# TheMTank/GridUniverse

Hardware: AMD Instinct MI355X
Metric: env-steps/sec at N_envs on 32×32 grid, 1/2/4/8 MI355X; bit-exact vs CPU (higher is better)
Workload: dtype int32; 1 GPU; c3: 65536 envs per GPU on the 32x32 generator maze (random.seed(123); np.random.seed(123)), uniform device-RNG actions, auto-reset, 1000 env-steps per launch, int32 (obs,reward,done) rows; envs_per_gpu=65536, env_steps_per_launch=1000, global_envs=65536, parallelism=env-index shards, no data-path collective

## Files before the change

### griduniverse_amd/csrc/gu_map.hpp

```cpp
#pragma once
#include "gu_internal.hpp"
#include "gu_rng.hpp"

#define GU_BLOCK 256

struct CellMap {
    const uint8_t *f;
    const int8_t *r;
};

__device__ __forceinline__ uint32_t gu_block_grid(const GridSel &gs)
{
    if (gs.n_grids <= 1) return 0u;
    const int64_t first = (int64_t)blockIdx.x * blockDim.x + (gs.per_wave ? (int64_t)(threadIdx.x & ~63u) : 0);
    const int64_t grid = first / gs.group;
    return (uint32_t)(grid < gs.n_grids ? grid : gs.n_grids - 1);
}

template <bool LDS>
__device__ __forceinline__ CellMap gu_stage_map(const uint8_t *__restrict__ g, int32_t cell_bytes, uint8_t *smem, const GridSel &gs,
                                                int planes = 2)
{
    if (LDS) {
        g += (int64_t)gu_block_grid(gs) * gs.grid_stride;
        if (gs.per_wave) {
            smem += (threadIdx.x >> 6) * (uint32_t)(planes * cell_bytes);
            for (int32_t i = (threadIdx.x & 63) * 16; i < planes * cell_bytes; i += 64 * 16)
                *reinterpret_cast<uint4 *>(smem + i) = *reinterpret_cast<const uint4 *>(g + i);
        } else {
            for (int32_t i = threadIdx.x * 16; i < planes * cell_bytes; i += blockDim.x * 16)
                *reinterpret_cast<uint4 *>(smem + i) = *reinterpret_cast<const uint4 *>(g + i);
        }
        __syncthreads();
        return CellMap{smem, reinterpret_cast<const int8_t *>(smem + cell_bytes)};
    }
    return CellMap{g, reinterpret_cast<const int8_t *>(g + cell_bytes)};
}

struct LaneGrid {
    const int32_t *starts;
    uint32_t n_starts;
};

template <bool LDS>
__device__ __forceinline__ LaneGrid gu_lane_grid(const GridSel &gs, const int32_t *starts, uint32_t n_starts0, uint32_t e, CellMap &m)
{
    if (gs.n_grids <= 1) return LaneGrid{starts, n_starts0};
    if (LDS) {
        const uint32_t gb = gu_block_grid(gs);
        return LaneGrid{starts + (int64_t)gb * gs.max_starts, (uint32_t)gs.n_starts[gb]};
    }
    const uint32_t g = e / (uint32_t)gs.group;
    m.f += (int64_t)g * gs.grid_stride;
    m.r += (int64_t)g * gs.grid_stride;
    return LaneGrid{starts + (int64_t)g * gs.max_starts, (uint32_t)gs.n_starts[g]};
}

template <bool LUT>
__device__ __forceinline__ int32_t gu_delta(uint32_t a, uint64_t lut, int32_t W)
{
    if (LUT) return __builtin_amdgcn_sbfe((int32_t)(uint32_t)(lut >> (a << 4)), 0, 16);
    const int32_t sign = (int32_t)(a & 2u) - 1;
    return (a & 1u) ? -sign : sign * W;
}

__device__ __forceinline__ int32_t gu_reward_packed(uint32_t flags)
{
    return __builtin_amdgcn_sbfe((int32_t)0xF6F60AFFu, (flags >> 2) & 24u, 8);
}

__device__ __forceinline__ int32_t gu_move(int32_t s, uint32_t flags, uint32_t a, int32_t delta)
{
    return __mul24((int32_t)__builtin_amdgcn_ubfe(flags, a, 1), delta) + s;
}
```

### griduniverse_amd/csrc/gu_rollout.hpp

```cpp
#pragma once
#include "gu_map.hpp"

#include <cstdlib>
#include <functional>
#include <type_traits>

__device__ __forceinline__ uint32_t gu_sample_action(uint32_t word, const uint4 q)
{
    return (uint32_t)(word >= q.x) + (uint32_t)(word >= q.y) + (uint32_t)(word >= q.z) - q.w;
}


#define GU_DPP_REDUCE(x, OP)                                                                                     \
    do {                                                                                                         \
        uint32_t o_;                                                                                             \
        o_ = (uint32_t)__builtin_amdgcn_update_dpp(0, (int)(x), 0x111, 0xF, 0xF, false), (x) = OP((x), o_);      \
        o_ = (uint32_t)__builtin_amdgcn_update_dpp(0, (int)(x), 0x112, 0xF, 0xF, false), (x) = OP((x), o_);      \
        o_ = (uint32_t)__builtin_amdgcn_update_dpp(0, (int)(x), 0x114, 0xF, 0xF, false), (x) = OP((x), o_);      \
        o_ = (uint32_t)__builtin_amdgcn_update_dpp(0, (int)(x), 0x118, 0xF, 0xF, false), (x) = OP((x), o_);      \
        o_ = (uint32_t)__builtin_amdgcn_update_dpp(0, (int)(x), 0x142, 0xA, 0xF, false), (x) = OP((x), o_);      \
        o_ = (uint32_t)__builtin_amdgcn_update_dpp(0, (int)(x), 0x143, 0xC, 0xF, false), (x) = OP((x), o_);      \
    } while (0)
#define GU_OP_ADD(a_, b_) ((a_) + (b_))
#define GU_OP_MAX(a_, b_) ((a_) > (b_) ? (a_) : (b_))

struct GuPacer {
    uint64_t due, t0;
    uint32_t ticks;
    uint32_t report_at;
    uint32_t n_steps;
    uint32_t p_q;
    uint64_t *slot;
    uint64_t w[16];
    uint32_t c_seq, c_phase, c_left, c_ema_p, c_ema_u, v_period_q, v_seq, v_unpaced, v_report_steps, v_groups;
    uint32_t c_dec_q, c_block_left, c_block_sum, c_block_n, c_last_mean, c_up, c_quiet;
    uint64_t v_t_start;
    bool first_wave;
    __device__ __forceinline__ void fetch(const GuPaceArgs &pa, bool on)
    {
        ticks = on ? pa.period : 0u;
        p_q = pa.period << 6;
        first_wave = false;
        if (on && pa.ring) {
            const GuPaceEntry *entry = pa.ring + (pa.seq & (GU_PACE_RING - 1u));
            const GuPaceEntry *prev = pa.ring + ((pa.seq - 1u) & (GU_PACE_RING - 1u));
            c_seq = entry->seq;
            const bool mine = c_seq == pa.seq;
            const uint32_t have = mine ? entry->period_q : 0u;
            const uint32_t unpaced = mine ? entry->unpaced : 0u;
            c_phase = entry->phase, c_left = entry->left, c_ema_p = entry->ema_paced, c_ema_u = entry->ema_unpaced;
            v_period_q = prev->period_q, v_seq = prev->seq, v_unpaced = prev->unpaced, v_t_start = prev->t_start;
            v_report_steps = prev->report_steps, v_groups = prev->groups;
            if (have && !pa.fixed) p_q = have;
            p_q = p_q < (pa.lo << 6) ? (pa.lo << 6) : p_q;
            p_q = p_q > (pa.hi << 6) ? (pa.hi << 6) : p_q;
            if (pa.fixed) p_q = pa.period << 6;
            ticks = (unpaced && !pa.fixed) ? 0u : (p_q + 32u) >> 6;
            c_quiet = (mine && !pa.fixed) ? entry->quiet : 0u;
            first_wave = blockIdx.x == 0 && __builtin_amdgcn_readfirstlane(threadIdx.x) < 64u;
            if (first_wave && !c_quiet) {
                c_dec_q = entry->dec_q, c_block_left = entry->block_left, c_block_sum = entry->block_sum, c_block_n = entry->block_n;
                c_last_mean = entry->last_mean, c_up = entry->up;
                const uint64_t *set = pa.slots + (size_t)((pa.seq - 1u) & 1u) * pa.slot_stride;
#pragma unroll
                for (uint32_t j = 0; j < 16u; ++j) {
                    const uint32_t i = j * 64u + threadIdx.x;
                    w[j] = i < pa.n_waves ? __builtin_nontemporal_load(set + i) : 0ull;
                }
            }
        }
    }
    __device__ __forceinline__ void start(const GuPaceArgs &pa, bool on)
    {
        slot = nullptr;
        n_steps = 0;
        report_at = 0;
        t0 = 0;
        if (on && pa.ring) {
            const uint64_t now = __builtin_amdgcn_s_memrealtime();
            due = t0 = now;
            if (c_quiet) {
                if (first_wave) decide_quiet(pa, now);
                return;
            }
            const uint32_t wave = __builtin_amdgcn_readfirstlane((blockIdx.x * blockDim.x + threadIdx.x) >> 6);
            slot = pa.slots + (size_t)(pa.seq & 1u) * pa.slot_stride + wave;
            report_at = pa.report_at;
            if (first_wave) decide(pa, now);
            return;
        }
        due = ticks ? __builtin_amdgcn_s_memrealtime() : 0ull;
    }
    __device__ __forceinline__ void decide_early(const GuPaceArgs &pa)
    {
        if (first_wave && !c_quiet) decide(pa, __builtin_amdgcn_s_memrealtime());
    }
    __device__ __forceinline__ void decide_quiet(const GuPaceArgs &pa, uint64_t now)
    {
        first_wave = false;
        if (threadIdx.x == 0) {
            GuPaceEntry *cur = pa.ring + (pa.seq & (GU_PACE_RING - 1u));
            GuPaceEntry *next = pa.ring + ((pa.seq + 1u) & (GU_PACE_RING - 1u));
            uint32_t ema_u = c_ema_u;
            const uint64_t gap = now - v_t_start;
            const uint32_t took = gap > 0x7FFFFFFFull ? 0x7FFFFFFFu : (uint32_t)gap;
            if (v_seq + 1u == pa.seq && v_unpaced && v_t_start && v_groups == pa.groups && (!ema_u || took < 2u * ema_u)) ema_u = ema_u ? (ema_u * 7u + took) >> 3 : took;
            cur->t_start = now, cur->groups = pa.groups, cur->report_steps = 0;
            const uint32_t left = c_left > 0u ? c_left - 1u : 0u;
            next->period_q = p_q, next->seq = pa.seq + 1u, next->t_start = 0, next->unpaced = 1u;
            next->phase = GU_PACE_OFF, next->left = left, next->ema_paced = c_ema_p, next->ema_unpaced = ema_u;
            next->verdict = 0, next->waves = 0, next->elapsed = 0, next->ended_late = 0, next->max_behind = 0, next->report_steps = 0, next->groups = 0;
            next->dec_q = pa.dec_q, next->block_left = GU_PACE_BLOCK, next->block_sum = 0, next->block_n = 0, next->last_mean = 0, next->up = 0;
            next->quiet = left > 1u ? 1u : 0u;
        }
    }
    __device__ __forceinline__ void decide(const GuPaceArgs &pa, uint64_t now)
    {
        first_wave = false;
        uint64_t *set = pa.slots + (size_t)((pa.seq - 1u) & 1u) * pa.slot_stride;
        GuPaceEntry *cur = pa.ring + (pa.seq & (GU_PACE_RING - 1u));
        GuPaceEntry *prev = pa.ring + ((pa.seq - 1u) & (GU_PACE_RING - 1u));
        const bool fresh = c_seq != pa.seq;
        const bool prev_ok = v_seq + 1u == pa.seq;
        const uint32_t prev_ticks = (prev_ok && !v_unpaced) ? (pa.fixed ? pa.period : (v_period_q + 32u) >> 6) : 0u;
        const uint32_t scheduled = (prev_ticks * ((v_report_steps + 15u) & ~15u)) >> 4;
        const bool same_length = v_groups == pa.groups;
        uint32_t counts = 0, most = 0, longest = 0;
        for (uint32_t base = 0; base < pa.n_waves; base += 64u * 16u) {
            if (base) {
#pragma unroll
                for (uint32_t j = 0; j < 16u; ++j) {
                    const uint32_t i = base + j * 64u + threadIdx.x;
                    w[j] = i < pa.n_waves ? __builtin_nontemporal_load(set + i) : 0ull;
                }
            }
#pragma unroll
            for (uint32_t j = 0; j < 16u; ++j) {
                const uint32_t i = base + j * 64u + threadIdx.x;
                if (i < pa.n_waves) set[i] = 0;
                const uint32_t reported = (uint32_t)(w[j] >> 63), elapsed = (uint32_t)w[j] & 0x7FFFFFFFu;
                const uint32_t behind = (prev_ticks && elapsed > scheduled) ? elapsed - scheduled : 0u;
                counts += (reported << 16) + ((reported && behind > 2u * prev_ticks) ? 1u : 0u);
                most = behind > most ? behind : most;
                longest = elapsed > longest ? elapsed : longest;
            }
        }
        GU_DPP_REDUCE(counts, GU_OP_ADD);
        GU_DPP_REDUCE(most, GU_OP_MAX);
        GU_DPP_REDUCE(longest, GU_OP_MAX);
        if (threadIdx.x == 63) {
            const uint32_t waves = counts >> 16, far = counts & 0xFFFFu;
            GuPaceEntry *next = pa.ring + ((pa.seq + 1u) & (GU_PACE_RING - 1u));
            uint32_t n_q = p_q, phase = GU_PACE_NORMAL, left = pa.probe_every ? (pa.probe_every < 128u ? pa.probe_every : 128u) : 0u, ema_p = 0, ema_u = 0;
            uint32_t dec_q = pa.dec_q, block_left = GU_PACE_BLOCK, block_sum = 0, block_n = 0, last_mean = 0, up = 0;
            if (!fresh) {
                phase = c_phase, left = c_left, ema_p = c_ema_p, ema_u = c_ema_u;
                dec_q = c_dec_q, block_left = c_block_left, block_sum = c_block_sum, block_n = c_block_n, last_mean = c_last_mean, up = c_up;
            } else {
                cur->unpaced = 0, cur->phase = phase, cur->left = left, cur->ema_paced = 0, cur->ema_unpaced = 0;
                cur->dec_q = dec_q, cur->block_left = block_left, cur->block_sum = 0, cur->block_n = 0, cur->last_mean = 0, cur->up = up;
            }
            cur->period_q = p_q, cur->seq = pa.seq, cur->t_start = now, cur->report_steps = pa.report_at, cur->groups = pa.groups;
            cur->verdict = 0, cur->waves = 0, cur->elapsed = 0, cur->ended_late = 0, cur->max_behind = 0;
            if (waves && prev_ok) {
                prev->verdict = (uint64_t)most * 256u > (uint64_t)prev_ticks * v_groups * pa.bar_num ? 2u : 1u;
                prev->waves = waves, prev->elapsed = longest, prev->ended_late = far, prev->max_behind = far ? most : 0u;
                const uint64_t gap = now - v_t_start;
                const uint32_t mean = v_unpaced ? ema_u : ema_p;
                const uint32_t took = gap > 0x7FFFFFFFull ? 0x7FFFFFFFu : (uint32_t)gap;
                const bool plausible = same_length && v_t_start && (!mean || took < 2u * mean);
                if (v_unpaced) {
                    if (plausible) ema_u = ema_u ? (ema_u + took) >> 1 : took;
                } else {
                    if (plausible) ema_p = ema_p ? (ema_p * 7u + took) >> 3 : took;
                    const uint32_t step_up = (uint32_t)(((uint64_t)pa.gain_q * far) / waves);
                    const uint32_t early = 512u / (8u + (pa.seq > 100000u ? 100000u : pa.seq));
                    const uint32_t dec = early > dec_q ? early : dec_q;
                    n_q += step_up;
                    n_q = n_q > dec ? n_q - dec : n_q;
                    if (phase == GU_PACE_NORMAL && !pa.fixed && pa.adapt) {
                        if (block_left <= GU_PACE_BLOCK - GU_PACE_BLOCK_SKIP && plausible) block_sum += took, ++block_n;
                        if (block_left) --block_left;
                        if (!block_left) {
                            const uint32_t mean = block_n ? block_sum / block_n : 0u;
                            if (mean && last_mean && mean > last_mean) up ^= 1u;
                            if (mean) last_mean = mean;
                            dec_q = up ? (dec_q * 4u + 2u) / 3u : (dec_q * 3u) / 4u;
                            dec_q = dec_q < 4u ? 4u : dec_q;
                            dec_q = dec_q > pa.gain_q / 8u ? pa.gain_q / 8u : dec_q;
                            block_left = GU_PACE_BLOCK, block_sum = 0, block_n = 0;
                        }
                    }
                }
            }
            n_q = n_q < (pa.lo << 6) ? (pa.lo << 6) : n_q;
            n_q = n_q > (pa.hi << 6) ? (pa.hi << 6) : n_q;
            if (pa.probe_every && !pa.fixed && left && --left == 0u) {
                const bool off_wins = ema_u && ema_p && (uint64_t)ema_u * 100u < (uint64_t)ema_p * 98u;
                if (phase != GU_PACE_NORMAL || off_wins) block_left = GU_PACE_BLOCK, block_sum = 0, block_n = 0, last_mean = 0;
                if (phase == GU_PACE_NORMAL) phase = GU_PACE_PROBE_OFF, left = 4u, ema_u = 0u;
                else if (phase == GU_PACE_OFF) phase = GU_PACE_PROBE_ON, left = 8u, ema_p = 0u;
                else if (off_wins) phase = GU_PACE_OFF, left = 2u * pa.probe_every;
                else phase = GU_PACE_NORMAL, left = pa.probe_every;
            }
            next->period_q = n_q, next->seq = pa.seq + 1u, next->t_start = 0;
            next->unpaced = (phase == GU_PACE_PROBE_OFF || phase == GU_PACE_OFF) ? 1u : 0u;
            next->phase = phase, next->left = left, next->ema_paced = ema_p, next->ema_unpaced = ema_u;
            next->dec_q = dec_q, next->block_left = block_left, next->block_sum = block_sum, next->block_n = block_n, next->last_mean = last_mean, next->up = up;
            next->quiet = (phase == GU_PACE_OFF && left > 1u) ? 1u : 0u;
            next->verdict = 0, next->waves = 0, next->elapsed = 0, next->ended_late = 0, next->max_behind = 0, next->report_steps = 0, next->groups = 0;
        }
    }
    __device__ __forceinline__ void report(uint64_t now)
    {
        if ((threadIdx.x & 63u) == 0u) {
            const uint64_t elapsed = now - t0;
            *slot = (1ull << 63) | (elapsed > 0x7FFFFFFFull ? 0x7FFFFFFFull : elapsed);
        }
        report_at = 0;
    }
    __device__ __forceinline__ bool idle() const { return ticks == 0u && slot == nullptr; }
    __device__ __forceinline__ void after(uint32_t steps)
    {
// ... 27 lines not shown
    uint32_t *episode;
    const uint32_t *tcount;
    const int32_t *starts;
    const uint32_t *actions;
    int32_t *tr_obs, *tr_reward, *tr_done;
    int32_t *ret, *episodes_fin;
    uint64_t *done_bits;
    uint32_t n_starts, seed_prefix, env_id0, steps_taken;
    uint32_t seed_prefix0, steps_hi;
    const uint32_t *nib;
    int32_t nib_dwords;
    uint64_t lut_p;
    int32_t straddle;
    int64_t N, T;
    GridSel gs;
    const uint32_t *rows;
    const uint32_t *rows2;
    int32_t row_shift;
    int32_t stream_lds_off;
    int32_t stream_lds_words;
    int32_t entry_table;
    int32_t half_waves;
    int32_t xcd_remap;
    GuPaceArgs pace;
};

__device__ __forceinline__ uint32_t gu_env_block(int32_t xcd_remap)
{
    const uint32_t b = blockIdx.x;
    return xcd_remap ? (b & 7u) * (gridDim.x >> 3) + (b >> 3) : b;
}

template <bool TAIL16 = false, class S16, class S1>
__device__ __forceinline__ void gu_stream_run(const char *pa, int64_t row, uint32_t e4, int64_t T, int64_t i0, S16 &&step16, S1 &&step1)
{
    const uint32_t row32 = (uint32_t)row;
    auto word_at = [&](int64_t k, uint32_t c) {
        return (uint32_t)__builtin_amdgcn_raw_buffer_load_b32(__builtin_amdgcn_make_buffer_rsrc((void *)(pa + k * row), 0, 0xFFFFFFFFu, 0x00020000), e4,
                                                              c * row32, 0);
    };
    int64_t i = i0, k = i0 >> 4;
    if (i & 15) {
        const uint32_t word = word_at(k, 0);
        for (; i < T && (i & 15); ++i) step1((word >> (2u * (uint32_t)(i & 15))) & 3u);
        ++k;
    }
    uint32_t w[4];
#pragma unroll
    for (uint32_t c = 0; c < 4; ++c) w[c] = word_at(k, c);
    for (const int64_t full = T >> 4; k + 4 <= full; k += 4, i += 64) {
#pragma unroll
        for (uint32_t c = 0; c < 4; ++c) {
            const uint32_t word = w[c];
            asm volatile("" ::"v"(word));
            w[c] = word_at(k + 4, c);
            step16(word);
        }
    }
    uint32_t q = 0;
    if (TAIL16) {
        for (; i + 16 <= T; i += 16, q += 16) {
            const uint32_t sel = q >> 4;
            step16(sel == 0 ? w[0] : sel == 1 ? w[1] : w[2]);
        }
    }
    for (; i < T; ++i, ++q) {
        const uint32_t sel = q >> 4, word = sel == 0 ? w[0] : sel == 1 ? w[1] : sel == 2 ? w[2] : w[3];
        step1((word >> (2u * (q & 15u))) & 3u);
    }
}

#ifndef GU_STORE_AUX
#define GU_STORE_AUX 18
#endif
#ifndef GU_STORE_AUX_PACKED
#define GU_STORE_AUX_PACKED 16
#endif
#define GU_MAX_BLOCK 1024
typedef uint32_t gu_v3u __attribute__((ext_vector_type(3)));
template <int POLICY, int AUTO, int TRAJ, bool STATS, int MAP>
__global__ void __launch_bounds__(GU_MAX_BLOCK) gu_rollout_kernel(const RolloutArgs a)
{
    constexpr bool LDS = MAP == 1 || MAP == 3;
    extern __shared__ __attribute__((aligned(16))) uint8_t smem[];
    GuPacer pacer;
    pacer.fetch(a.pace, TRAJ == 1 || TRAJ == 3);
    const int64_t e64 = (int64_t)gu_env_block(a.xcd_remap) * blockDim.x + threadIdx.x;
    const bool live = e64 < a.N;
    const uint32_t e = (uint32_t)e64;
    int32_t s = 0, r = 0;
    uint32_t d = 0, ep = 0, tcount0 = 0;
    if (live) {
        s = a.pos[e];
        r = a.reward[e];
        d = (uint32_t)a.done[e];
        ep = a.episode[e];
        tcount0 = a.tcount[e];
    }
    CellMap m = gu_stage_map<LDS>(a.cell, a.cell_bytes, smem, a.gs, MAP == 3 ? 1 : 2);
    const uint32_t nib_region = MAP == 5 ? (threadIdx.x >> 6) * (uint32_t)a.nib_dwords * 256u : 0u;
    if (MAP == 5) {
        const size_t wave = ((size_t)blockIdx.x * blockDim.x + threadIdx.x) >> 6;
        const uint4 *src = reinterpret_cast<const uint4 *>(a.nib + wave * (size_t)a.nib_dwords * 64u);
        uint4 *dst = reinterpret_cast<uint4 *>(smem + nib_region);
        if (wave * 64u < (size_t)a.N)
            for (int32_t i = threadIdx.x & 63; i < a.nib_dwords * 16; i += 64) dst[i] = src[i];
        __syncthreads();
    }
    const uint8_t *greedy = a.greedy;
    if (MAP == 1 && POLICY == GU_POLICY_GREEDY) {
        uint8_t *dst = smem + 2 * a.cell_bytes;
        for (int32_t i = threadIdx.x * 16; i < a.cell_bytes; i += blockDim.x * 16)
            *reinterpret_cast<uint4 *>(dst + i) = *reinterpret_cast<const uint4 *>(a.greedy + i);
        __syncthreads();
        greedy = dst;
    }
    const bool thr_in_lds = MAP == 1 && POLICY == GU_POLICY_SAMPLE && a.pi_lds;
    uint4 *thr_lds = reinterpret_cast<uint4 *>(smem + 2 * a.cell_bytes);
    if (thr_in_lds) {
        for (int32_t i = threadIdx.x; i < a.S; i += blockDim.x) thr_lds[i] = a.pi_thr[i];
        __syncthreads();
    }
    if (!live) return;
    LaneGrid lg = gu_lane_grid<LDS>(a.gs, a.starts, a.n_starts, e, m);

    const uint32_t t_lane = tcount0 + a.steps_taken;
    const uint32_t prefix = gu_rng_prefix(a.seed_prefix, a.env_id0 + e);
    const uint32_t prefix0 = AUTO == 2 ? gu_rng_prefix(a.seed_prefix0, a.env_id0 + e) : prefix;
    const uint32_t epoch0 = (uint32_t)((uint64_t)((int64_t)(((uint64_t)a.steps_hi << 32) | a.steps_taken) + (int64_t)(int32_t)tcount0) >> 32);
    auto prefix_at = [&](uint32_t t) {
        return gu_rng_prefix(gu_rng_seed_prefix_epoch(a.seed_prefix0, epoch0 + (t < t_lane ? 1u : 0u)), a.env_id0 + e);
    };
    constexpr uint32_t TERM5 = 0x20u, TERM5_BIT = 5u;
    auto flags5 = [](uint32_t b) { return (((b >> 5) & 3u) << 3) | (((b >> GU_CELL_TERM_BIT) & 1u) << TERM5_BIT) | ((b >> 7) << 6); };
    uint32_t flags = MAP == 5 ? flags5(m.f[s]) : m.f[s];
    int32_t ret = 0, fin = 0;
    const int32_t W = a.W;
    const uint64_t lut = a.lut;
    const int32_t start0 = lg.starts[0];
    const uint32_t start0_flags = MAP == 5 ? flags5(m.f[start0]) : m.f[start0];
    auto padded = [&](int32_t c) { return (int32_t)(((uint32_t)(c + c / W + W + 2) << 5) + nib_region); };
    int32_t sq = MAP == 5 ? padded(s) : 0;
    const int32_t start0_q = MAP == 5 ? padded(start0) : 0;
    typedef __attribute__((address_space(3))) const uint32_t *lds_word_ptr;
    const uint32_t lane4 = (threadIdx.x & 63u) << 2;
    auto word_at = [&](int32_t cq) { return *(lds_word_ptr)(uintptr_t)(((uint32_t)cq & 0xFFFFFF00u) | lane4); };
    auto four_of = [](uint32_t word, int32_t cq) { return __builtin_amdgcn_ubfe(word, (uint32_t)cq >> 3, 4); };
    auto four_at = [&](int32_t cq) { return four_of(word_at(cq), cq); };
    auto cell5 = [&](int32_t cq) { return four_at(cq) << 3; };
    auto move5 = [&](uint32_t act, int32_t delta, auto &&in_the_shadow) {
        int32_t cand = s + delta;
        asm volatile("" : "+v"(cand));
        const int32_t candq = sq + gu_delta<true>(act, a.lut_p, 0);
        const uint32_t word = word_at(candq);
        in_the_shadow();
        const uint32_t four = four_of(word, candq);
        const bool go = ((flags & TERM5) | four) < 8u;
        s = go ? cand : s;
        sq = go ? candq : sq;
        flags = go ? four << 3 : flags;
    };
    char *po = (char *)a.tr_obs, *pr = (char *)a.tr_reward, *pd = (char *)a.tr_done;
    const char *pa = (const char *)a.actions;
    const uint32_t e4 = e * 4u;
    const int64_t row = a.N * 4;
    const uint32_t row32 = (uint32_t)row;
    const int64_t trow = TRAJ == 3 ? a.N * 12 : row;
    const uint32_t trow32 = (uint32_t)trow;
    const uint32_t te = TRAJ == 3 ? e * 12u : e4;
    __amdgpu_buffer_rsrc_t ro = __builtin_amdgcn_make_buffer_rsrc(po, 0, 0xFFFFFFFFu, 0x00020000);
    __amdgpu_buffer_rsrc_t rr = __builtin_amdgcn_make_buffer_rsrc(pr, 0, 0xFFFFFFFFu, 0x00020000);
    __amdgpu_buffer_rsrc_t rd = __builtin_amdgcn_make_buffer_rsrc(pd, 0, 0xFFFFFFFFu, 0x00020000);
    auto emit = [&](int32_t s_, int32_t r_, uint32_t d_, uint32_t soff) {
        if (TRAJ == 1) {
            __builtin_amdgcn_raw_buffer_store_b32(s_, ro, e4, soff, GU_STORE_AUX);
            __builtin_amdgcn_raw_buffer_store_b32(r_, rr, e4, soff, GU_STORE_AUX);
            __builtin_amdgcn_raw_buffer_store_b32((int32_t)d_, rd, e4, soff, GU_STORE_AUX);
        } else if (TRAJ == 2) {
            __builtin_amdgcn_raw_buffer_store_b32((int32_t)((uint32_t)s_ | (((uint32_t)r_ & 0xFFu) << 16) | (d_ << 24)), ro, e4, soff, GU_STORE_AUX_PACKED);
        } else if (TRAJ == 3) {
            const gu_v3u triple = {(uint32_t)s_, (uint32_t)r_, d_};
            __builtin_amdgcn_raw_buffer_store_b96(triple, ro, te, soff, GU_STORE_AUX);
            GU_WIDE_STORE_PAD();
        }
    };
    bool held = false;
    int32_t held_s = 0, held_r = 0;
    uint32_t held_d = 0, held_soff = 0;
    auto release = [&]() {
        if (MAP == 5 && TRAJ && held) emit(held_s, held_r, held_d, held_soff);
        held = false;
    };
    auto rebase = [&](int64_t rows) {
        release();
        po += rows * trow;
        ro = __builtin_amdgcn_make_buffer_rsrc(po, 0, 0xFFFFFFFFu, 0x00020000);
        if (TRAJ == 1) {
            pr += rows * trow;
            pd += rows * trow;
            rr = __builtin_amdgcn_make_buffer_rsrc(pr, 0, 0xFFFFFFFFu, 0x00020000);
            rd = __builtin_amdgcn_make_buffer_rsrc(pd, 0, 0xFFFFFFFFu, 0x00020000);
        }
    };

    if (AUTO == 1 && MAP != 5) flags = (flags & ~GU_CELL_TERM) | (d << GU_CELL_TERM_BIT);

    auto step = [&](uint32_t act, uint32_t soff) {
        const int32_t delta = gu_delta<MAP != 0>(act, lut, W);
        if (AUTO == 1) {
            const bool was_done = MAP == 5 ? d != 0u : (flags & GU_CELL_TERM) != 0u;
            ep += was_done;
            s = was_done ? start0 : s;
            flags = was_done ? start0_flags : flags;
            if (MAP == 5) sq = was_done ? start0_q : sq;
        } else if (AUTO == 2) {
            if (d) {
                s = lg.starts[gu_rng_start_index(prefix0, ep, lg.n_starts)];
                ++ep;
                if (MAP == 5) sq = padded(s);
                flags = MAP == 5 ? cell5(sq) : m.f[s];
            }
        }
        if (MAP == 5) {
            move5(act, delta, [&]() {
                if (TRAJ && held) {
                    __builtin_amdgcn_sched_barrier(0);
                    emit(held_s, held_r, held_d, held_soff);
                    __builtin_amdgcn_sched_barrier(0);
                }
            });
        } else {
            s = gu_move(s, flags, act, delta);
            flags = m.f[s];
        }
        r = MAP == 5 ? __builtin_amdgcn_sbfe((int32_t)0xF6F60AFFu, flags, 8) : (MAP >= 2) ? gu_reward_packed(flags) : (int32_t)m.r[s];
        d = __builtin_amdgcn_ubfe(flags, MAP == 5 ? TERM5_BIT : GU_CELL_TERM_BIT, 1);
        if (STATS) {
            ret += r;
            fin += (int32_t)d;
        }
        if (MAP == 5 && TRAJ) held = true, held_s = s, held_r = r, held_d = d, held_soff = soff;
        else emit(s, r, d, soff);
    };
    auto step1 = [&](uint32_t act) {
        step(act, 0);
        if (TRAJ) rebase(1);
    };

    pacer.start(a.pace, TRAJ == 1 || TRAJ == 3);
    if (POLICY == GU_POLICY_UNIFORM && a.straddle) {
        uint32_t t = t_lane;
#pragma nounroll
        for (int64_t i = 0; i < a.T; ++i, ++t) step1((gu_rng_word(prefix_at(t), GU_RNG_STREAM_ACTION, t >> 4) >> (2u * (t & 15u))) & 3u);
    } else if (POLICY == GU_POLICY_UNIFORM) {
        const uint32_t t_first = __builtin_amdgcn_readfirstlane(t_lane);
        if (__all(t_lane == t_first)) {
            uint32_t t = t_first;
            int64_t i = 0;
            if (t & 15u) {
                const uint32_t word = gu_rng_word(prefix, GU_RNG_STREAM_ACTION, t >> 4);
                for (; i < a.T && (t & 7u); ++i, ++t) step1((word >> (2u * (t & 15u))) & 3u);
                if ((t & 15u) == 8u && i + 8 <= a.T) {
#pragma unroll
                    for (uint32_t j = 0; j < 8; ++j) step(__builtin_amdgcn_ubfe(word, 16 + 2 * j, 2), j * trow32);
                    if (TRAJ) rebase(8);
                    i += 8, t += 8;
                }
                for (; i < a.T && (t & 15u); ++i, ++t) step1((word >> (2u * (t & 15u))) & 3u);
                pacer.after((uint32_t)i);
            }
            for (; i + 16 <= a.T; i += 16, t += 16) {
                uint32_t word = gu_rng_word(prefix, GU_RNG_STREAM_ACTION, t >> 4);
                if (MAP == 5) asm volatile("" : "+v"(word));
#pragma unroll
                for (uint32_t j = 0; j < 16; ++j) step(__builtin_amdgcn_ubfe(word, 2 * j, 2), j * trow32);
                if (TRAJ) rebase(16);
                if (i + 16 < a.T) pacer.after(16);
            }
            if (i < a.T) {
                const uint32_t word = gu_rng_word(prefix, GU_RNG_STREAM_ACTION, t >> 4);
                uint32_t j = 0;
                if (i + 8 <= a.T) {
#pragma unroll
                    for (uint32_t k = 0; k < 8; ++k) step(__builtin_amdgcn_ubfe(word, 2 * k, 2), k * trow32);
                    if (TRAJ) rebase(8);
                    i += 8, j = 8;
                }
                for (; i < a.T; ++i, ++j) step1((word >> (2u * j)) & 3u);
            }
        } else {
            uint32_t t = t_lane;
            uint32_t word = gu_rng_word(prefix, GU_RNG_STREAM_ACTION, t >> 4);
            for (int64_t i = 0; i < a.T; ++i) {
                step1((word >> (2u * (t & 15u))) & 3u);
                ++t;
                if ((t & 15u) == 0u) word = gu_rng_word(prefix, GU_RNG_STREAM_ACTION, t >> 4);
            }
        }
    } else if (POLICY == GU_POLICY_STREAM) {
        const char *pw = pa;
        auto load_word = [&](uint32_t soff) {
            return (uint32_t)__builtin_amdgcn_raw_buffer_load_b32(__builtin_amdgcn_make_buffer_rsrc((void *)pw, 0, 0xFFFFFFFFu, 0x00020000), e4, soff, 0);
        };
        const int64_t KW = (MAP == 1) ? a.stream_lds_words : 0;
        if (KW) {
            uint32_t *sw = reinterpret_cast<uint32_t *>(smem + a.stream_lds_off) + threadIdx.x;
            const uint32_t bd = blockDim.x;
            int64_t words_left = (a.T + 15) >> 4, i = 0;
            while (i < a.T) {
                const int64_t cnt = words_left < KW ? words_left : KW;
                int64_t k = 0;
                for (; k + 8 <= cnt; k += 8) {
                    uint32_t w[8];
#pragma unroll
                    for (int j = 0; j < 8; ++j) w[j] = load_word(j * row32);
#pragma unroll
                    for (int j = 0; j < 8; ++j) sw[(k + j) * bd] = w[j];
                    pw += 8 * row;
                }
                for (; k < cnt; ++k, pw += row) sw[k * bd] = load_word(0);
                words_left -= cnt;
                const int64_t steps = (a.T - i) < cnt * 16 ? (a.T - i) : cnt * 16;
                uint32_t word = sw[0];
                for (k = 0; k * 16 + 16 <= steps; ++k) {
                    const uint32_t next = k + 1 < cnt ? sw[(k + 1) * bd] : 0u;
#pragma unroll
                    for (uint32_t j = 0; j < 16; ++j) step(__builtin_amdgcn_ubfe(word, 2 * j, 2), j * trow32);
                    if (TRAJ) rebase(16);
                    pacer.after(16);
                    word = next;
                }
                for (int64_t q = k * 16, j = 0; q < steps; ++q, ++j) step1((word >> (2u * (uint32_t)j)) & 3u);
// ... 227 lines not shown
```

### griduniverse_amd/csrc/gu_rollout_rows.hip

```cpp
#include "gu_rollout.hpp"

#define GU_ROW_ADDR_MASK 0xFFFFFu
#define GU_ROW_DONE_BIT 23

struct BuildRowsArgs {
    const uint8_t *cell;
    int32_t cell_bytes, S, W, start0, auto_reset, row_shift;
    uint32_t *rows;
};

__global__ void __launch_bounds__(256) gu_build_rows_kernel(const BuildRowsArgs a)
{
    const int32_t s = blockIdx.x * blockDim.x + threadIdx.x;
    if (s >= a.S) return;
    const int32_t base = (a.auto_reset && (a.cell[s] & GU_CELL_TERM)) ? a.start0 : s;
    const uint32_t fb = a.cell[base];
    uint32_t out[4];
#pragma unroll
    for (uint32_t act = 0; act < 4; ++act) {
        const int32_t n = base + (((fb >> act) & 1u) ? gu_delta<false>(act, 0, a.W) : 0);
        const uint32_t d = (a.cell[n] >> GU_CELL_TERM_BIT) & 1u;
        const uint32_t r = (uint8_t)a.cell[a.cell_bytes + n];
        out[act] = ((uint32_t)n << a.row_shift) | (d << GU_ROW_DONE_BIT) | (r << 24);
    }
// ... 15 lines not shown
    const uint32_t d = (cell[n] >> GU_CELL_TERM_BIT) & 1u;
    const uint32_t r = (uint8_t)cell[cell_bytes + n];
    return ((uint32_t)n << row_shift) | (d << GU_ROW_DONE_BIT) | (r << 24);
}

__global__ void __launch_bounds__(256) gu_build_policy_rows_kernel(const BuildPolicyRowsArgs a)
{
    const int32_t s = blockIdx.x * blockDim.x + threadIdx.x;
    if (s >= a.S) return;
    const int32_t base = (a.auto_reset && (a.cell[s] & GU_CELL_TERM)) ? a.start0 : s;
    if (!a.thr) {
        a.rows[s] = gu_row_record(a.cell, a.cell_bytes, base, a.greedy[base], a.W, a.row_shift);
        return;
    }
    uint4 *out = reinterpret_cast<uint4 *>(a.rows + 8 * (int64_t)s);
    const uint4 q = a.thr[base];
    uint32_t t0 = q.x, t1 = q.y, t2 = q.z;
    if (t0 > t1) { const uint32_t x = t0; t0 = t1; t1 = x; }
    if (t1 > t2) { const uint32_t x = t1; t1 = t2; t2 = x; }
    if (t0 > t1) { const uint32_t x = t0; t0 = t1; t1 = x; }
    out[0] = make_uint4(t0, t1, t2, q.w);
    uint32_t rec[4];
#pragma unroll
    for (uint32_t c = 0; c < 4; ++c) {
        const uint32_t act = c >= q.w ? (c - q.w > 3u ? 3u : c - q.w) : 0u;
        rec[c] = gu_row_record(a.cell, a.cell_bytes, base, act, a.W, a.row_shift);
    }
    out[1] = make_uint4(rec[0], rec[1], rec[2], rec[3]);
}

__device__ __forceinline__ uint32_t gu_row_record(const uint8_t *cell, int32_t cell_bytes, int32_t base, uint32_t act, int32_t W, int32_t row_shift);

struct BuildPairRowsArgs {
    const uint8_t *cell;
    int32_t cell_bytes, S, W, start0, auto_reset;
    uint32_t *rows2;
};

#define GU_PAIR_SHIFT 7

__global__ void __launch_bounds__(256) gu_build_pair_rows_kernel(const BuildPairRowsArgs a)
{
    const int32_t idx = blockIdx.x * blockDim.x + threadIdx.x;
    if (idx >= a.S * 16) return;
    const int32_t s = idx >> 4;
    const uint32_t a1 = (uint32_t)idx & 3u, a2 = ((uint32_t)idx >> 2) & 3u;
    const int32_t b1 = (a.auto_reset && (a.cell[s] & GU_CELL_TERM)) ? a.start0 : s;
    const uint32_t r1 = gu_row_record(a.cell, a.cell_bytes, b1, a1, a.W, GU_PAIR_SHIFT);
    const int32_t n1 = (int32_t)((r1 & GU_ROW_ADDR_MASK) >> GU_PAIR_SHIFT);
    const int32_t b2 = (a.auto_reset && (a.cell[n1] & GU_CELL_TERM)) ? a.start0 : n1;
    const uint32_t r2 = gu_row_record(a.cell, a.cell_bytes, b2, a2, a.W, GU_PAIR_SHIFT);
    reinterpret_cast<uint2 *>(a.rows2)[idx] = make_uint2(r1, r2);
}

typedef __attribute__((address_space(3))) const uint32_t *lds_u32_ptr;
typedef uint32_t gu_v2u __attribute__((ext_vector_type(2)));
typedef __attribute__((address_space(3))) const gu_v2u *lds_v2u_ptr;
typedef uint32_t gu_v4u __attribute__((ext_vector_type(4)));
typedef __attribute__((address_space(3))) const gu_v4u *lds_v4u_ptr;

template <int POLICY>
struct RowBytes {
    static constexpr int log2 = POLICY == GU_POLICY_GREEDY ? 2 : POLICY == GU_POLICY_SAMPLE ? 5 : 4;
};

#define GU_CHAIN_FENCE() __builtin_amdgcn_sched_barrier(0)
#define GU_ROWS_MAX_BLOCK 512
template <int POLICY, int TRAJ, bool STATS, bool PAIR = false>
__global__ void __launch_bounds__(GU_ROWS_MAX_BLOCK) gu_rollout_rows_kernel(const RolloutArgs a, const int32_t auto_reset)
{
    static_assert(!PAIR || POLICY == GU_POLICY_UNIFORM || POLICY == GU_POLICY_STREAM, "pair tables: policies whose actions do not depend on the state");
    extern __shared__ __attribute__((aligned(16))) uint8_t smem[];
    GuPacer pacer;
    pacer.fetch(a.pace, TRAJ != 0);
    const int32_t shift = PAIR ? GU_PAIR_SHIFT : a.row_shift;
    const int32_t copies_log2 = shift - RowBytes<POLICY>::log2;
    constexpr uint32_t lds_base = 0u;
    const uint32_t half = (uint32_t)a.half_waves;
    const uint32_t slot_in_block = half ? ((threadIdx.x >> 6) << 5) | (threadIdx.x & 31u) : threadIdx.x;
    const int64_t e64 = (int64_t)gu_env_block(a.xcd_remap) * (blockDim.x >> half) + slot_in_block;
    const bool live = e64 < a.N && !(half && (threadIdx.x & 32u));
    const uint32_t e = live ? (uint32_t)e64 : 0u;
    const uint32_t prefix = gu_rng_prefix(a.seed_prefix, a.env_id0 + e);
    const int32_t start0 = auto_reset ? a.starts[0] : 0;
    const char *pa = (const char *)a.actions;
    const uint32_t e4 = e * 4u;
    int32_t s = 0;
    uint32_t d = 0, ep = 0, t_lane = 0, f0 = 0, first_x = 0, f1 = 0, r1 = 0, first_word = 0;
    uint4 first_thr = make_uint4(0u, 0u, 0u, 0u);
    auto first_0 = [&]() {
        uint32_t ee = e;
        asm volatile("" : "+v"(ee));
        s = a.pos[ee];
        d = (uint32_t)a.done[ee];
        ep = a.episode[ee];
        t_lane = a.tcount[ee];
    };
    const bool entry_table = a.entry_table != 0;
    auto first_a = [&]() {
        asm volatile("" : "+v"(t_lane), "+v"(s), "+v"(d));
        t_lane += a.steps_taken;
        if (POLICY == GU_POLICY_SAMPLE) first_word = gu_rng_sample_word(prefix, t_lane);
        if (auto_reset && d) {
            if (!entry_table) s = start0;
            ++ep;
        }
        if (!entry_table) {
            f0 = a.cell[s];
            if (POLICY == GU_POLICY_GREEDY) first_x = a.greedy[s];
            if (POLICY == GU_POLICY_SAMPLE) first_thr = a.pi_thr[s];
        }
        if (POLICY == GU_POLICY_UNIFORM) first_x = (gu_rng_word(prefix, GU_RNG_STREAM_ACTION, t_lane >> 4) >> (2u * (t_lane & 15u))) & 3u;
        if (POLICY == GU_POLICY_STREAM) first_x = (uint32_t)__builtin_amdgcn_raw_buffer_load_b32(__builtin_amdgcn_make_buffer_rsrc((void *)pa, 0, 0xFFFFFFFFu, 0x00020000), e4, 0, 0) & 3u;
    };
    auto first_b = [&]() {
        if (entry_table) return;
        asm volatile("" : "+v"(f0));
        const uint32_t act = POLICY == GU_POLICY_SAMPLE ? gu_sample_action(first_word, first_thr) : first_x;
        const int8_t *rew = reinterpret_cast<const int8_t *>(a.cell + a.cell_bytes);
        s += ((f0 >> act) & 1u) ? gu_delta<false>(act, 0, a.W) : 0;
        f1 = a.cell[s];
        r1 = (uint32_t)(uint8_t)rew[s];
    };
    {
        uint4 *dst = reinterpret_cast<uint4 *>(smem);
        const uint32_t copies = 1u << copies_log2;
        if (POLICY == GU_POLICY_GREEDY && copies_log2 < 2) {
            const int32_t units = (a.S << shift) >> 4;
            first_0();
            first_a();
#pragma unroll 8
            for (int32_t u = threadIdx.x; u < units; u += blockDim.x) {
                const int32_t d0 = u << 2;
                uint4 v = make_uint4(a.rows[d0 >> copies_log2], a.rows[(d0 + 1) >> copies_log2], a.rows[(d0 + 2) >> copies_log2], a.rows[(d0 + 3) >> copies_log2]);
                v.x += lds_base, v.y += lds_base, v.z += lds_base, v.w += lds_base;
                dst[u] = v;
            }
            first_b();
        } else {
            const int32_t B = (int32_t)blockDim.x, log2_b = 31 - __builtin_clz((uint32_t)B);
            const int32_t n_src = PAIR ? a.S * 9 : POLICY == GU_POLICY_SAMPLE ? 2 * a.S : a.S;
            const uint4 *g4 = reinterpret_cast<const uint4 *>(PAIR ? a.rows2 : a.rows);
            const uint32_t places = PAIR ? 1u : POLICY == GU_POLICY_GREEDY ? copies >> 2 : copies;
            auto put = [&](uint4 v, int32_t g) {
                if (PAIR || (POLICY != GU_POLICY_GREEDY && (POLICY != GU_POLICY_SAMPLE || (g & 1)))) v.x += lds_base, v.y += lds_base, v.z += lds_base, v.w += lds_base;
                if (PAIR) {
                    dst[g] = v;
                    return;
                }
                const uint32_t cell = POLICY == GU_POLICY_SAMPLE ? (uint32_t)g >> 1 : (uint32_t)g;
                auto at = [&](uint32_t k) {
                    const uint32_t place = (k + cell) & (places - 1u);
                    return POLICY == GU_POLICY_SAMPLE ? ((cell * places + place) << 1) | ((uint32_t)g & 1u) : cell * places + place;
                };
                if (places == 8u) {
#pragma unroll
                    for (uint32_t k = 0; k < 8u; ++k) dst[at(k)] = v;
                } else if (places == 4u) {
#pragma unroll
                    for (uint32_t k = 0; k < 4u; ++k) dst[at(k)] = v;
                } else {
                    for (uint32_t k = 0; k < places; ++k) dst[at(k)] = v;
                }
            };
            auto stage = [&](auto nb, int32_t base, auto between) {
                constexpr int NB = decltype(nb)::value;
                uint4 v[NB];
// ... 442 lines not shown
```

### griduniverse_amd/csrc/gu_rollout_uniform.hip

```cpp
#include "gu_rollout.hpp"

void gu_rollout_uniform(gu_engine *h, const RolloutArgs &a, int auto_mode, int traj, bool stats, int bs)
{
    gu_rollout_dispatch<GU_POLICY_UNIFORM>(h, a, auto_mode, traj, stats, bs);
}
```

Before: 590.1 billion env-steps/s.

## Overlap kernel prologue loads: split map staging into issue/finish, buffer loads for pacer

Kernel prologue loads are restructured so global reads are issued early and consumed later. Map, table and nibble staging into LDS is split into an issue phase of buffer loads and a finish phase. The pacer record is now fetched as one coalesced per-lane load and unpacked with readlane. Start-state loads go through buffer loads to a scalar-friendly path. The goal is to hide prologue memory latency ahead of the step loop, at the cost of more live registers and more complex pacer-state handling, plus optional timing-stamp instrumentation.

```diff
diff --git a/griduniverse_amd/csrc/gu_map.hpp b/griduniverse_amd/csrc/gu_map.hpp
--- a/griduniverse_amd/csrc/gu_map.hpp
+++ b/griduniverse_amd/csrc/gu_map.hpp
@@ -12,29 +12,82 @@
 __device__ __forceinline__ uint32_t gu_block_grid(const GridSel &gs)
 {
     if (gs.n_grids <= 1) return 0u;
-    const int64_t first = (int64_t)blockIdx.x * blockDim.x + (gs.per_wave ? (int64_t)(threadIdx.x & ~63u) : 0);
+    const uint32_t wave0 = gs.per_wave ? __builtin_amdgcn_readfirstlane(threadIdx.x & ~63u) : 0u;
+    const int64_t first = (int64_t)blockIdx.x * blockDim.x + (int64_t)wave0;
     const int64_t grid = first / gs.group;
-    return (uint32_t)(grid < gs.n_grids ? grid : gs.n_grids - 1);
+    return __builtin_amdgcn_readfirstlane((uint32_t)(grid < gs.n_grids ? grid : gs.n_grids - 1));
+}
+
+typedef uint32_t gu_v4u __attribute__((ext_vector_type(4)));
+struct GuStage {
+    gu_v4u v0, v1;
+    __device__ __forceinline__ void load(const void *src, int32_t first, int32_t stride, int32_t n)
+    {
+        __amdgpu_buffer_rsrc_t rs = __builtin_amdgcn_make_buffer_rsrc(const_cast<void *>(src), 0, n * 16, 0x00020000);
+        v0 = __builtin_amdgcn_raw_buffer_load_b128(rs, first * 16, 0, 0);
+        v1 = __builtin_amdgcn_raw_buffer_load_b128(rs, (first + stride) * 16, 0, 0);
+    }
+    __device__ __forceinline__ void put(void *dst, int32_t first, int32_t stride, int32_t n) const
+    {
+        gu_v4u *d = reinterpret_cast<gu_v4u *>(dst);
+        if (first < n) d[first] = v0;
+        if (first + stride < n) d[first + stride] = v1;
+    }
+    __device__ __forceinline__ void finish(const void *src, void *dst, int32_t first, int32_t stride, int32_t n)
+    {
+        put(dst, first, stride, n);
+        for (int32_t i = first + 2 * stride; i < n; i += 2 * stride) {
+            load(src, i, stride, n);
+            put(dst, i, stride, n);
+        }
+    }
+};
+
+struct MapStage {
+    GuStage st;
+    const uint8_t *src;
+    uint8_t *smem;
+    int32_t first, stride, n;
+};
+
+template <bool LDS>
+__device__ __forceinline__ MapStage gu_stage_map_issue(const uint8_t *__restrict__ g, int32_t cell_bytes, uint8_t *smem, const GridSel &gs,
+                                                       uint32_t grid, int planes = 2)
+{
+    MapStage ms;
+    ms.src = g + (int64_t)grid * gs.grid_stride;
+    ms.smem = smem;
+    ms.first = 0, ms.stride = 0, ms.n = 0;
+    if (LDS) {
+        ms.n = (planes * cell_bytes + 15) >> 4;
+        if (gs.per_wave) {
+            ms.smem = smem + (threadIdx.x >> 6) * (uint32_t)(planes * cell_bytes);
+            ms.first = (int32_t)(threadIdx.x & 63u), ms.stride = 64;
+        } else {
+            ms.first = (int32_t)threadIdx.x, ms.stride = (int32_t)blockDim.x;
+        }
+        ms.st.load(ms.src, ms.first, ms.stride, ms.n);
+    }
+    return ms;
+}
+
+template <bool LDS>
+__device__ __forceinline__ CellMap gu_stage_map_finish(MapStage &ms, int32_t cell_bytes)
+{
+    if (LDS) {
+        ms.st.finish(ms.src, ms.smem, ms.first, ms.stride, ms.n);
+        __syncthreads();
+        return CellMap{ms.smem, reinterpret_cast<const int8_t *>(ms.smem + cell_bytes)};
+    }
+    return CellMap{ms.src, reinterpret_cast<const int8_t *>(ms.src + cell_bytes)};
 }
 
 template <bool LDS>
 __device__ __forceinline__ CellMap gu_stage_map(const uint8_t *__restrict__ g, int32_t cell_bytes, uint8_t *smem, const GridSel &gs,
                                                 int planes = 2)
 {
-    if (LDS) {
-        g += (int64_t)gu_block_grid(gs) * gs.grid_stride;
-        if (gs.per_wave) {
-            smem += (threadIdx.x >> 6) * (uint32_t)(planes * cell_bytes);
-            for (int32_t i = (threadIdx.x & 63) * 16; i < planes * cell_bytes; i += 64 * 16)
-                *reinterpret_cast<uint4 *>(smem + i) = *reinterpret_cast<const uint4 *>(g + i);
-        } else {
-            for (int32_t i = threadIdx.x * 16; i < planes * cell_bytes; i += blockDim.x * 16)
-                *reinterpret_cast<uint4 *>(smem + i) = *reinterpret_cast<const uint4 *>(g + i);
-        }
-        __syncthreads();
-        return CellMap{smem, reinterpret_cast<const int8_t *>(smem + cell_bytes)};
-    }
-    return CellMap{g, reinterpret_cast<const int8_t *>(g + cell_bytes)};
+    MapStage ms = gu_stage_map_issue<LDS>(g, cell_bytes, smem, gs, LDS ? gu_block_grid(gs) : 0u, planes);
+    return gu_stage_map_finish<LDS>(ms, cell_bytes);
 }
 
 struct LaneGrid {
@@ -42,14 +95,22 @@
     uint32_t n_starts;
 };
 
+__device__ __forceinline__ uint32_t gu_load_word_vmem(const void *p)
+{
+    return (uint32_t)__builtin_amdgcn_raw_buffer_load_b32(__builtin_amdgcn_make_buffer_rsrc(const_cast<void *>(p), 0, 4, 0x00020000), 0, 0, 0);
+}
+
+__device__ __forceinline__ LaneGrid gu_block_starts(const GridSel &gs, const int32_t *starts, uint32_t n_starts0, uint32_t grid)
+{
+    if (gs.n_grids <= 1) return LaneGrid{starts, n_starts0};
+    return LaneGrid{starts + (int64_t)grid * gs.max_starts, gu_load_word_vmem(gs.n_starts + grid)};
+}
+
 template <bool LDS>
 __device__ __forceinline__ LaneGrid gu_lane_grid(const GridSel &gs, const int32_t *starts, uint32_t n_starts0, uint32_t e, CellMap &m)
 {
+    if (LDS) return gu_block_starts(gs, starts, n_starts0, gu_block_grid(gs));
     if (gs.n_grids <= 1) return LaneGrid{starts, n_starts0};
-    if (LDS) {
-        const uint32_t gb = gu_block_grid(gs);
-        return LaneGrid{starts + (int64_t)gb * gs.max_starts, (uint32_t)gs.n_starts[gb]};
-    }
     const uint32_t g = e / (uint32_t)gs.group;
     m.f += (int64_t)g * gs.grid_stride;
     m.r += (int64_t)g * gs.grid_stride;
diff --git a/griduniverse_amd/csrc/gu_rollout.hpp b/griduniverse_amd/csrc/gu_rollout.hpp
--- a/griduniverse_amd/csrc/gu_rollout.hpp
+++ b/griduniverse_amd/csrc/gu_rollout.hpp
@@ -4,6 +4,20 @@
 #include <cstdlib>
 #include <functional>
 #include <type_traits>
+
+#ifdef GU_STAMP_PROLOGUE
+#define GU_STAMP_WAVES 4096
+static __device__ uint32_t gu_stamp_ticks[GU_STAMP_WAVES];
+#define GU_STAMP_ENTRY() const uint64_t gu_t_entry = __builtin_amdgcn_s_memrealtime()
+#define GU_STAMP_START(pacer_)                                                                              \
+    do {                                                                                                    \
+        const uint32_t wave_ = (blockIdx.x * blockDim.x + threadIdx.x) >> 6;                                \
+        if ((threadIdx.x & 63u) == 0u && wave_ < GU_STAMP_WAVES && (pacer_).t0) gu_stamp_ticks[wave_] = (uint32_t)((pacer_).t0 - gu_t_entry); \
+    } while (0)
+#else
+#define GU_STAMP_ENTRY()
+#define GU_STAMP_START(pacer_)
+#endif
 
 __device__ __forceinline__ uint32_t gu_sample_action(uint32_t word, const uint4 q)
 {
@@ -31,47 +45,75 @@
     uint32_t n_steps;
     uint32_t p_q;
     uint64_t *slot;
-    uint64_t w[16];
+    typedef uint32_t v2u __attribute__((ext_vector_type(2)));
+    v2u w[16];
+    bool packed;
+    uint32_t rec;
     uint32_t c_seq, c_phase, c_left, c_ema_p, c_ema_u, v_period_q, v_seq, v_unpaced, v_report_steps, v_groups;
     uint32_t c_dec_q, c_block_left, c_block_sum, c_block_n, c_last_mean, c_up, c_quiet;
     uint64_t v_t_start;
-    bool first_wave;
+    bool first_wave, armed;
+    __device__ __forceinline__ void load_slots(const GuPaceArgs &pa, const uint64_t *set, uint32_t base)
+    {
+        __amdgpu_buffer_rsrc_t rs = __builtin_amdgcn_make_buffer_rsrc(const_cast<uint64_t *>(set), 0, (int)(pa.n_waves * 8u), 0x00020000);
+#pragma unroll
+        for (uint32_t j = 0; j < 16u; ++j) w[j] = __builtin_amdgcn_raw_buffer_load_b64(rs, (int)((base + j * 64u + threadIdx.x) * 8u), 0, 2);
+        packed = false;
+    }
+    __device__ __forceinline__ void pack()
+    {
+        if (!packed) {
+#pragma unroll
+            for (uint32_t j = 0; j < 16u; ++j) w[j].x = (w[j].x & 0x7FFFFFFFu) | (w[j].y & 0x80000000u);
+        }
+        packed = true;
+    }
     __device__ __forceinline__ void fetch(const GuPaceArgs &pa, bool on)
     {
         ticks = on ? pa.period : 0u;
         p_q = pa.period << 6;
         first_wave = false;
-        if (on && pa.ring) {
+        c_seq = 0, c_quiet = 0, rec = 0;
+        packed = true;
+        armed = on && pa.ring;
+        if (armed) {
             const GuPaceEntry *entry = pa.ring + (pa.seq & (GU_PACE_RING - 1u));
             const GuPaceEntry *prev = pa.ring + ((pa.seq - 1u) & (GU_PACE_RING - 1u));
-            c_seq = entry->seq;
+            rec = reinterpret_cast<const uint32_t *>((threadIdx.x & 32u) ? prev : entry)[threadIdx.x & 31u];
+            first_wave = blockIdx.x == 0 && __builtin_amdgcn_readfirstlane(threadIdx.x) < 64u;
+            if (first_wave) load_slots(pa, pa.slots + (size_t)((pa.seq - 1u) & 1u) * pa.slot_stride, 0u);
+        }
+    }
+#define GU_REC(lane0, field) ((uint32_t)__builtin_amdgcn_readlane((int)rec, (lane0) + (int)(offsetof(GuPaceEntry, field) / 4)))
+    __device__ __forceinline__ void unpack()
+    {
+        c_phase = GU_REC(0, phase), c_left = GU_REC(0, left), c_ema_p = GU_REC(0, ema_paced), c_ema_u = GU_REC(0, ema_unpaced);
+        c_dec_q = GU_REC(0, dec_q), c_block_left = GU_REC(0, block_left), c_block_sum = GU_REC(0, block_sum), c_block_n = GU_REC(0, block_n);
+        c_last_mean = GU_REC(0, last_mean), c_up = GU_REC(0, up);
+        v_period_q = GU_REC(32, period_q), v_seq = GU_REC(32, seq), v_unpaced = GU_REC(32, unpaced);
+        v_t_start = ((uint64_t)GU_REC(33, t_start) << 32) | GU_REC(32, t_start);
+        v_report_steps = GU_REC(32, report_steps), v_groups = GU_REC(32, groups);
+    }
+    __device__ __forceinline__ void settle(const GuPaceArgs &pa)
+    {
+        if (armed) {
+            c_seq = GU_REC(0, seq);
             const bool mine = c_seq == pa.seq;
-            const uint32_t have = mine ? entry->period_q : 0u;
-            const uint32_t unpaced = mine ? entry->unpaced : 0u;
-            c_phase = entry->phase, c_left = entry->left, c_ema_p = entry->ema_paced, c_ema_u = entry->ema_unpaced;
-            v_period_q = prev->period_q, v_seq = prev->seq, v_unpaced = prev->unpaced, v_t_start = prev->t_start;
-            v_report_steps = prev->report_steps, v_groups = prev->groups;
+            const uint32_t have = mine ? GU_REC(0, period_q) : 0u;
+            const uint32_t unpaced = mine ? GU_REC(0, unpaced) : 0u;
+            p_q = pa.period << 6;
             if (have && !pa.fixed) p_q = have;
             p_q = p_q < (pa.lo << 6) ? (pa.lo << 6) : p_q;
             p_q = p_q > (pa.hi << 6) ? (pa.hi << 6) : p_q;
             if (pa.fixed) p_q = pa.period << 6;
             ticks = (unpaced && !pa.fixed) ? 0u : (p_q + 32u) >> 6;
-            c_quiet = (mine && !pa.fixed) ? entry->quiet : 0u;
-            first_wave = blockIdx.x == 0 && __builtin_amdgcn_readfirstlane(threadIdx.x) < 64u;
-            if (first_wave && !c_quiet) {
-                c_dec_q = entry->dec_q, c_block_left = entry->block_left, c_block_sum = entry->block_sum, c_block_n = entry->block_n;
-                c_last_mean = entry->last_mean, c_up = entry->up;
-                const uint64_t *set = pa.slots + (size_t)((pa.seq - 1u) & 1u) * pa.slot_stride;
-#pragma unroll
-                for (uint32_t j = 0; j < 16u; ++j) {
-                    const uint32_t i = j * 64u + threadIdx.x;
-                    w[j] = i < pa.n_waves ? __builtin_nontemporal_load(set + i) : 0ull;
-                }
-            }
-        }
-    }
+            c_quiet = (mine && !pa.fixed) ? GU_REC(0, quiet) : 0u;
+        }
+    }
+#undef GU_REC
     __device__ __forceinline__ void start(const GuPaceArgs &pa, bool on)
     {
+        settle(pa);
         slot = nullptr;
         n_steps = 0;
         report_at = 0;
@@ -93,11 +135,13 @@
     }
     __device__ __forceinline__ void decide_early(const GuPaceArgs &pa)
     {
+        settle(pa);
         if (first_wave && !c_quiet) decide(pa, __builtin_amdgcn_s_memrealtime());
     }
     __device__ __forceinline__ void decide_quiet(const GuPaceArgs &pa, uint64_t now)
     {
         first_wave = false;
+        unpack();
         if (threadIdx.x == 0) {
             GuPaceEntry *cur = pa.ring + (pa.seq & (GU_PACE_RING - 1u));
             GuPaceEntry *next = pa.ring + ((pa.seq + 1u) & (GU_PACE_RING - 1u));
@@ -116,7 +160,9 @@
     }
     __device__ __forceinline__ void decide(const GuPaceArgs &pa, uint64_t now)
     {
+        pack();
         first_wave = false;
+        unpack();
         uint64_t *set = pa.slots + (size_t)((pa.seq - 1u) & 1u) * pa.slot_stride;
         GuPaceEntry *cur = pa.ring + (pa.seq & (GU_PACE_RING - 1u));
         GuPaceEntry *prev = pa.ring + ((pa.seq - 1u) & (GU_PACE_RING - 1u));
@@ -127,18 +173,12 @@
         const bool same_length = v_groups == pa.groups;
         uint32_t counts = 0, most = 0, longest = 0;
         for (uint32_t base = 0; base < pa.n_waves; base += 64u * 16u) {
-            if (base) {
-#pragma unroll
-                for (uint32_t j = 0; j < 16u; ++j) {
-                    const uint32_t i = base + j * 64u + threadIdx.x;
-                    w[j] = i < pa.n_waves ? __builtin_nontemporal_load(set + i) : 0ull;
-                }
-            }
+            if (base) load_slots(pa, set, base), pack();
 #pragma unroll
             for (uint32_t j = 0; j < 16u; ++j) {
                 const uint32_t i = base + j * 64u + threadIdx.x;
                 if (i < pa.n_waves) set[i] = 0;
-                const uint32_t reported = (uint32_t)(w[j] >> 63), elapsed = (uint32_t)w[j] & 0x7FFFFFFFu;
+                const uint32_t reported = w[j].x >> 31, elapsed = w[j].x & 0x7FFFFFFFu;
                 const uint32_t behind = (prev_ticks && elapsed > scheduled) ? elapsed - scheduled : 0u;
                 counts += (reported << 16) + ((reported && behind > 2u * prev_ticks) ? 1u : 0u);
                 most = behind > most ? behind : most;
@@ -332,6 +372,7 @@
 __global__ void __launch_bounds__(GU_MAX_BLOCK) gu_rollout_kernel(const RolloutArgs a)
 {
     constexpr bool LDS = MAP == 1 || MAP == 3;
+    GU_STAMP_ENTRY();
     extern __shared__ __attribute__((aligned(16))) uint8_t smem[];
     GuPacer pacer;
     pacer.fetch(a.pace, TRAJ == 1 || TRAJ == 3);
@@ -347,32 +388,43 @@
         ep = a.episode[e];
         tcount0 = a.tcount[e];
     }
-    CellMap m = gu_stage_map<LDS>(a.cell, a.cell_bytes, smem, a.gs, MAP == 3 ? 1 : 2);
-    const uint32_t nib_region = MAP == 5 ? (threadIdx.x >> 6) * (uint32_t)a.nib_dwords * 256u : 0u;
-    if (MAP == 5) {
-        const size_t wave = ((size_t)blockIdx.x * blockDim.x + threadIdx.x) >> 6;
-        const uint4 *src = reinterpret_cast<const uint4 *>(a.nib + wave * (size_t)a.nib_dwords * 64u);
-        uint4 *dst = reinterpret_cast<uint4 *>(smem + nib_region);
-        if (wave * 64u < (size_t)a.N)
-            for (int32_t i = threadIdx.x & 63; i < a.nib_dwords * 16; i += 64) dst[i] = src[i];
-        __syncthreads();
-    }
-    const uint8_t *greedy = a.greedy;
-    if (MAP == 1 && POLICY == GU_POLICY_GREEDY) {
-        uint8_t *dst = smem + 2 * a.cell_bytes;
-        for (int32_t i = threadIdx.x * 16; i < a.cell_bytes; i += blockDim.x * 16)
-            *reinterpret_cast<uint4 *>(dst + i) = *reinterpret_cast<const uint4 *>(a.greedy + i);
-        __syncthreads();
-        greedy = dst;
-    }
+    const uint32_t grid = LDS ? gu_block_grid(a.gs) : 0u;
+    LaneGrid lg = gu_block_starts(a.gs, a.starts, a.n_starts, grid);
+    int32_t start0 = 0;
+    if (LDS) start0 = (int32_t)gu_load_word_vmem(lg.starts);
+    MapStage ms = gu_stage_map_issue<LDS>(a.cell, a.cell_bytes, smem, a.gs, grid, MAP == 3 ? 1 : 2);
+    const bool greedy_in_lds = MAP == 1 && POLICY == GU_POLICY_GREEDY;
     const bool thr_in_lds = MAP == 1 && POLICY == GU_POLICY_SAMPLE && a.pi_lds;
     uint4 *thr_lds = reinterpret_cast<uint4 *>(smem + 2 * a.cell_bytes);
-    if (thr_in_lds) {
-        for (int32_t i = threadIdx.x; i < a.S; i += blockDim.x) thr_lds[i] = a.pi_thr[i];
+    const void *table = greedy_in_lds ? (const void *)a.greedy : (const void *)a.pi_thr;
+    const int32_t table_n = greedy_in_lds ? a.cell_bytes >> 4 : thr_in_lds ? a.S : 0;
+    GuStage ts;
+    if (greedy_in_lds || thr_in_lds) ts.load(table, (int32_t)threadIdx.x, (int32_t)blockDim.x, table_n);
+    const uint32_t nib_region = MAP == 5 ? (threadIdx.x >> 6) * (uint32_t)a.nib_dwords * 256u : 0u;
+    const size_t nib_wave = ((size_t)blockIdx.x * blockDim.x + __builtin_amdgcn_readfirstlane(threadIdx.x)) >> 6;
+    const int32_t nib_n = (MAP == 5 && nib_wave * 64u < (size_t)a.N) ? a.nib_dwords * 16 : 0;
+    const uint32_t *nib_src = a.nib + nib_wave * (size_t)a.nib_dwords * 64u;
+    GuStage ns;
+    if (MAP == 5) ns.load(nib_src, (int32_t)(threadIdx.x & 63u), 64, nib_n);
+    CellMap m = gu_stage_map_finish<false>(ms, a.cell_bytes);
+    if (!LDS && live) {
+        lg = gu_lane_grid<false>(a.gs, a.starts, a.n_starts, e, m);
+        start0 = lg.starts[0];
+    }
+    pacer.pack();
+    if (LDS) m = gu_stage_map_finish<true>(ms, a.cell_bytes);
+    if (MAP == 5) {
+        ns.finish(nib_src, smem + nib_region, (int32_t)(threadIdx.x & 63u), 64, nib_n);
         __syncthreads();
     }
+    const uint8_t *greedy = a.greedy;
+    if (greedy_in_lds || thr_in_lds) {
+        ts.finish(table, thr_lds, (int32_t)threadIdx.x, (int32_t)blockDim.x, table_n);
+        __syncthreads();
+        if (greedy_in_lds) greedy = smem + 2 * a.cell_bytes;
+    }
+    pacer.settle(a.pace);
     if (!live) return;
-    LaneGrid lg = gu_lane_grid<LDS>(a.gs, a.starts, a.n_starts, e, m);
 
     const uint32_t t_lane = tcount0 + a.steps_taken;
     const uint32_t prefix = gu_rng_prefix(a.seed_prefix, a.env_id0 + e);
@@ -387,7 +439,6 @@
     int32_t ret = 0, fin = 0;
     const int32_t W = a.W;
     const uint64_t lut = a.lut;
-    const int32_t start0 = lg.starts[0];
     const uint32_t start0_flags = MAP == 5 ? flags5(m.f[start0]) : m.f[start0];
     auto padded = [&](int32_t c) { return (int32_t)(((uint32_t)(c + c / W + W + 2) << 5) + nib_region); };
     int32_t sq = MAP == 5 ? padded(s) : 0;
@@ -498,6 +549,7 @@
     };
 
     pacer.start(a.pace, TRAJ == 1 || TRAJ == 3);
+    GU_STAMP_START(pacer);
     if (POLICY == GU_POLICY_UNIFORM && a.straddle) {
         uint32_t t = t_lane;
 #pragma nounroll
diff --git a/griduniverse_amd/csrc/gu_rollout_rows.hip b/griduniverse_amd/csrc/gu_rollout_rows.hip
--- a/griduniverse_amd/csrc/gu_rollout_rows.hip
+++ b/griduniverse_amd/csrc/gu_rollout_rows.hip
@@ -121,7 +121,7 @@
     const bool live = e64 < a.N && !(half && (threadIdx.x & 32u));
     const uint32_t e = live ? (uint32_t)e64 : 0u;
     const uint32_t prefix = gu_rng_prefix(a.seed_prefix, a.env_id0 + e);
-    const int32_t start0 = auto_reset ? a.starts[0] : 0;
+    const int32_t start0 = auto_reset ? (int32_t)gu_load_word_vmem(a.starts) : 0;
     const char *pa = (const char *)a.actions;
     const uint32_t e4 = e * 4u;
     int32_t s = 0;
diff --git a/griduniverse_amd/csrc/gu_rollout_uniform.hip b/griduniverse_amd/csrc/gu_rollout_uniform.hip
--- a/griduniverse_amd/csrc/gu_rollout_uniform.hip
+++ b/griduniverse_amd/csrc/gu_rollout_uniform.hip
@@ -4,3 +4,11 @@
 {
     gu_rollout_dispatch<GU_POLICY_UNIFORM>(h, a, auto_mode, traj, stats, bs);
 }
+
+#ifdef GU_STAMP_PROLOGUE
+extern "C" int gu_stamp_read(uint32_t *out, int n)
+{
+    if (n < 0 || n > GU_STAMP_WAVES) return -1;
+    return (int)hipMemcpyFromSymbol(out, HIP_SYMBOL(gu_stamp_ticks), (size_t)n * sizeof(uint32_t));
+}
+#endif
```

Result: no change. 591.5 billion env-steps/s (median of 2 runs) (+0.2%).
